# linnil1/KIR_graph

Hardware: AMD Instinct MI355X
Metric: typed 150 bp PE reads/s (pileup+EM) per GPU; achieved HBM GB/s vs roofline (higher is better)
Workload: dtype f64

## Files before the change

kir_graph_amd/csrc/gk_common.h:

```cpp
#pragma once
#include <hip/hip_runtime.h>
#include <hip/hip_ext.h>

#include <cstdarg>
#include <cstdint>
#include <cstdio>
#include <cstring>
#include <deque>
#include <map>
#include <mutex>
#include <unordered_map>
#include <vector>

#include "graphkir_hip.h"
#include "gk_env.h"

void gk_set_error(const char* fmt, ...);

#define GK_HIP(call)                                                                   \
  do {                                                                                 \
    hipError_t e_ = (call);                                                            \
    if (e_ != hipSuccess) {                                                            \
      gk_set_error("%s failed: %s (%s:%d)", #call, hipGetErrorString(e_), __FILE__, __LINE__); \
      return GK_ERR_HIP;                                                               \
// ... 88 lines not shown

struct gk_index {
  gk_ctx* ctx = nullptr;
  uint64_t* d_key = nullptr;
  int32_t* d_gene_vbeg = nullptr;
  int32_t* d_bucket = nullptr;
  int32_t* d_gene_boff = nullptr;
  uint32_t* d_del_bits = nullptr;
  int32_t* d_lb_a = nullptr;
  int32_t* d_lb_t = nullptr;
  int32_t* d_gene_pbase = nullptr;
  int32_t* d_snp_ord = nullptr;
  int32_t n_var = 0, n_gene = 0;
  std::vector<int32_t> gene_vbeg;
};

struct gk_tab {
  gk_ctx* ctx = nullptr;
  gk_index* idx = nullptr;
  int32_t n_var = 0;
  int64_t n_pairs = 0, n_valid = 0, n_ids = 0;
  int32_t n_novel = 0, err_flags = 0;
  int32_t* d_pair_src = nullptr;
  uint32_t* d_off = nullptr;
  uint32_t* d_ids = nullptr;
  uint8_t* d_pair_gene = nullptr;
  uint8_t* d_pair_nh = nullptr;
  uint64_t* d_novel_key = nullptr;
  gk_mate_wide* d_wide = nullptr;
  int64_t n_spill = 0;
  struct GenePartition {
    gk_ctx* owner = nullptr;
    int32_t* d_rows = nullptr;
    std::vector<int64_t> gene_off;
  } part[2];
  std::mutex part_mutex;
};

template <typename T>
static inline T* gk_ptr(gk_dptr p) {
  return reinterpret_cast<T*>(static_cast<uintptr_t>(p));
}
static inline gk_dptr gk_addr(const void* p) { return static_cast<gk_dptr>(reinterpret_cast<uintptr_t>(p)); }

int gk_scan_u32(gk_ctx* ctx, uint32_t* d_data, int64_t n, uint32_t* d_total);
int gk_compact_enqueue(gk_ctx* ctx, const uint32_t* d_flag, const int32_t* d_values, int64_t n, int32_t* d_out,
                       uint32_t** d_total_out, std::vector<void*>& temps);
int gk_compact(gk_ctx* ctx, const uint32_t* d_flag, const int32_t* d_values, int64_t n, int32_t* d_out,
               int64_t* n_out);

#define GK_KEY_REF_SHIFT 56
#define GK_KEY_POS_SHIFT 32
#define GK_KEY_TYP_SHIFT 30
#define GK_KEY_VAL_MASK 0x3FFFFFFFull
#define GK_TYP_INS 0ull
#define GK_TYP_SINGLE 1ull
#define GK_TYP_DEL 2ull
__host__ __device__ static inline uint64_t gk_make_key(uint32_t ref, uint32_t pos, uint64_t typ, uint32_t val) {
  return ((uint64_t)ref << GK_KEY_REF_SHIFT) | ((uint64_t)(pos & 0xFFFFFFu) << GK_KEY_POS_SHIFT) |
         (typ << GK_KEY_TYP_SHIFT) | ((uint64_t)val & GK_KEY_VAL_MASK);
}
__host__ __device__ static inline uint32_t gk_key_pos(uint64_t k) { return (uint32_t)(k >> GK_KEY_POS_SHIFT) & 0xFFFFFFu; }
__host__ __device__ static inline uint32_t gk_key_typ(uint64_t k) { return (uint32_t)(k >> GK_KEY_TYP_SHIFT) & 3u; }
__host__ __device__ static inline uint32_t gk_key_val(uint64_t k) { return (uint32_t)(k & GK_KEY_VAL_MASK); }
```

kir_graph_amd/csrc/gk_tabulate.hip:

```cpp
#include <algorithm>
#include <vector>

#include "gk_common.h"

namespace {

constexpr int kThreads = 256;
constexpr int kMaxEv = GK_MAX_EVENTS;
constexpr uint64_t kEmpty = ~0ull;

constexpr int kMateWords = sizeof(gk_mate) / 4;
constexpr int kCigWord = 3;
constexpr int kMmWord = kCigWord + GK_MAX_CIG / 2;
constexpr int kInsWord = kMmWord + GK_MAX_MM;
static_assert(sizeof(gk_mate) == 128 && kInsWord + GK_MAX_INS == kMateWords, "gk_mate layout");
constexpr int kRecLd = kMateWords + 1;
constexpr int kEvLd = kMaxEv + 1;
constexpr int kMaskWords = 8;

constexpr uint32_t kEvNovel = 1u << 31;
constexpr uint32_t kEvIsN = 1u << 30;
constexpr uint32_t kEvOrdMask = (1u << 26) - 1;
constexpr uint32_t kEvSlotMask = (1u << 30) - 1;

// ... 1045 lines not shown
  GK_HIP(gk_pool_malloc(ctx, (void**)&tab->d_off, (size_t)(4 * n_valid + 1) * sizeof(uint32_t)));
  GK_HIP(gk_pool_malloc(ctx, (void**)&tab->d_ids, (size_t)(n_ids + 1) * sizeof(uint32_t)));
  GK_HIP(gk_pool_malloc(ctx, (void**)&tab->d_pair_gene, (size_t)n_valid + 1));
  GK_HIP(gk_pool_malloc(ctx, (void**)&tab->d_pair_nh, (size_t)n_valid + 1));
  GK_HIP(hipMemcpyAsync(tab->d_off, off, (size_t)(4 * n_valid + 1) * sizeof(uint32_t), hipMemcpyHostToDevice, st));
  if (n_ids) GK_HIP(hipMemcpyAsync(tab->d_ids, ids, (size_t)n_ids * sizeof(uint32_t), hipMemcpyHostToDevice, st));
  if (n_valid) {
    GK_HIP(hipMemcpyAsync(tab->d_pair_gene, pair_gene, (size_t)n_valid, hipMemcpyHostToDevice, st));
    GK_HIP(hipMemcpyAsync(tab->d_pair_nh, pair_nh, (size_t)n_valid, hipMemcpyHostToDevice, st));
  }
  GK_HIP(hipStreamSynchronize(st));
  *out = tab;
  return GK_OK;
}

int gk_tab_get_info(gk_tab* tab, gk_tab_info* info) {
  gk_bind(tab ? tab->ctx : nullptr);
  GK_REQUIRE(tab && info, "null pointer");
  info->n_pairs = tab->n_pairs; info->n_valid = tab->n_valid; info->n_ids = tab->n_ids;
  info->n_novel = tab->n_novel; info->err_flags = tab->err_flags;
  info->d_pair_src = gk_addr(tab->d_pair_src); info->d_off = gk_addr(tab->d_off); info->d_ids = gk_addr(tab->d_ids);
  info->d_pair_gene = gk_addr(tab->d_pair_gene); info->d_pair_nh = gk_addr(tab->d_pair_nh);
  info->d_novel_key = gk_addr(tab->d_novel_key);
  return GK_OK;
}

int gk_tab_destroy(gk_tab* tab) {
  gk_bind(tab ? tab->ctx : nullptr);
  if (!tab) return GK_OK;
  gk_ctx* ctx = tab->ctx;
  gk_pool_free(ctx,tab->d_pair_src); gk_pool_free(ctx,tab->d_off); gk_pool_free(ctx,tab->d_ids);
  gk_pool_free(ctx,tab->d_pair_gene); gk_pool_free(ctx,tab->d_pair_nh); gk_pool_free(ctx,tab->d_novel_key);
  gk_pool_free(ctx,tab->d_wide);
  for (auto& part : tab->part)
    if (part.d_rows) gk_pool_free(part.owner, part.d_rows);
  delete tab;
  return GK_OK;
}

}

extern "C" {

int gk_mates_compact(gk_ctx* ctx, gk_dptr d_mates, int64_t n_mates, gk_dptr* d_compact_out, int64_t* bytes_out) {
  gk_bind(ctx);
  GK_REQUIRE(ctx && d_compact_out && bytes_out && n_mates >= 0 && (n_mates == 0 || d_mates), "bad compaction arguments");
  GK_REQUIRE(n_mates < (1ll << 27), "more than 2^26 pairs per call");
  hipStream_t st = ctx->stream;
  const gk_mate* mates = gk_ptr<const gk_mate>(d_mates);
  uint32_t* cnt = nullptr;
  GK_HIP(gk_pool_malloc(ctx, (void**)&cnt, (size_t)(n_mates + 2) * sizeof(uint32_t)));
  if (n_mates) GK_KERNEL(mates_count_words, dim3(nblk(n_mates)), dim3(kThreads), 0, st, mates, n_mates, cnt);
  int rc = gk_scan_u32(ctx, cnt, n_mates, cnt + n_mates);
  if (rc) { gk_pool_free(ctx, cnt); return rc; }
  uint32_t total = 0;
  GK_HIP(gk_fetch(ctx, &total, cnt + n_mates, sizeof(uint32_t)));
  const size_t bytes = ((size_t)(n_mates + 1) + (size_t)total) * sizeof(uint32_t);
  uint32_t* out = nullptr;
  GK_HIP(gk_pool_malloc(ctx, (void**)&out, bytes));
  GK_KERNEL(mates_pack_words, dim3(nblk(n_mates + 1)), dim3(kThreads), 0, st, mates, n_mates, cnt, out, out + n_mates + 1, total);
  GK_HIP(hipGetLastError());
  gk_pool_free(ctx, cnt);
  *d_compact_out = gk_addr(out);
  *bytes_out = (int64_t)bytes;
  return GK_OK;
}

int gk_mates_expand(gk_ctx* ctx, gk_dptr d_compact, int64_t n_mates, gk_dptr d_mates_out) {
// ... 12 lines not shown
```

kir_graph_amd/csrc/gk_typing.hip:

```cpp
#include <algorithm>

#include "gk_common.h"
#include "gk_lut.h"

namespace {

constexpr int kThreads = 256;
inline unsigned nblk(int64_t n, int t = kThreads) { return (unsigned)((n + t - 1) / t); }

template <bool kScatter>
__global__ __launch_bounds__(kThreads) void part_pass(const uint8_t* gene, const uint8_t* nh, int64_t n, int multiple,
                                                      int n_bins, int64_t n_tiles, uint32_t* hist, int32_t* out) {
  const int64_t i = (int64_t)blockIdx.x * kThreads + threadIdx.x;
  const int lane = threadIdx.x & 63;
  const int64_t tile = i >> 6;
  int bin = -1;
  if (i < n && (multiple || nh[i] == 1)) {
    bin = gene[i];
    if (bin >= n_bins) bin = -1;
  }
  uint64_t todo = __ballot(bin >= 0);
  while (todo) {
    const int leader = __ffsll((unsigned long long)todo) - 1;
    const int b = __shfl(bin, leader, 64);
// ... 14 lines not shown
}

__global__ __launch_bounds__(kThreads) void count_ids(const int32_t* __restrict__ rows, int64_t n_rows,
                                                      const uint32_t* __restrict__ off,
                                                      const uint32_t* __restrict__ ids,
                                                      const uint8_t* __restrict__ vflag, uint32_t* cnt_pos,
                                                      uint32_t* cnt_neg, int vbeg, int n_local) {
  extern __shared__ uint32_t hist[];
  for (int i = threadIdx.x; i < 2 * n_local; i += kThreads) hist[i] = 0;
  __syncthreads();
  constexpr int kGroup = 16;
  const int lane = threadIdx.x & (kGroup - 1);
  const int64_t group = ((int64_t)blockIdx.x * kThreads + threadIdx.x) / kGroup;
  const int64_t n_groups = ((int64_t)gridDim.x * kThreads) / kGroup;
  for (int64_t i = group; i < n_rows; i += n_groups) {
    const int64_t row = rows[i];
    const uint32_t b = off[4 * row], mid = off[4 * row + 2], e = off[4 * row + 4];
    for (uint32_t k = b + lane; k < e; k += kGroup) {
      const uint32_t v = ids[k];
      const bool positive = k < mid;
      if (vflag[v] & (positive ? 1 : 2)) continue;
      const uint32_t l = v - (uint32_t)vbeg;
      if (l < (uint32_t)n_local) atomicAdd(&hist[(positive ? 0 : n_local) + l], 1u);
      else atomicAdd(positive ? &cnt_pos[v] : &cnt_neg[v], 1u);
    }
  }
  __syncthreads();
  for (int i = threadIdx.x; i < 2 * n_local; i += kThreads) {
    const uint32_t c = hist[i];
    if (c) atomicAdd(i < n_local ? &cnt_pos[vbeg + i] : &cnt_neg[vbeg + i - n_local], c);
  }
}

__global__ __launch_bounds__(kThreads) void apply_correction(const uint32_t* cnt_pos, const uint32_t* cnt_neg,
                                                             int64_t n, uint8_t* vflag) {
  const int64_t v = (int64_t)blockIdx.x * kThreads + threadIdx.x;
  if (v >= n) return;
  const uint64_t p = cnt_pos[v], q = cnt_neg[v];
  if (p + q == 0) return;
  uint8_t f = vflag[v];
  if (p + q < 3) {
    f |= 3;
  } else {
    if (5 * p < p + q) f |= 1;
    if (5 * q < p + q) f |= 2;
  }
  vflag[v] = f;
}

__global__ __launch_bounds__(kThreads) void flag_nonempty(const int32_t* rows, int64_t n_rows, const uint32_t* off,
                                                          const uint32_t* ids, const uint8_t* vflag, uint32_t* flag,
                                                          uint32_t* zero, int n_zero) {
  const int64_t i = (int64_t)blockIdx.x * kThreads + threadIdx.x;
  if (zero && i < n_zero) zero[i] = 0;
  if (i >= n_rows) return;
  const int64_t row = rows[i];
  const uint32_t b = off[4 * row], mid = off[4 * row + 2], e = off[4 * row + 4];
  uint32_t alive = 0;
  for (uint32_t k = b; k < e && !alive; ++k) alive = !(vflag[ids[k]] & (k < mid ? 1 : 2));
  flag[i] = alive;
}

__global__ __launch_bounds__(kThreads) void flag_pairs(int64_t n_pairs, const uint32_t* __restrict__ off,
                                                       const uint32_t* __restrict__ ids, const uint8_t* __restrict__ vflag,
                                                       const uint8_t* __restrict__ maybe, uint8_t* __restrict__ alive) {
  const int64_t t = (int64_t)blockIdx.x * kThreads + threadIdx.x;
  const int64_t p = t >> 2;
  const uint32_t l = (uint32_t)t & 3u;
  uint32_t b = 0, mid = 0, e = 0;
  if (p < n_pairs && maybe[p]) { b = off[4 * p]; mid = off[4 * p + 2]; e = off[4 * p + 4]; }
  const int shift = (threadIdx.x & 63) & ~3;
  bool any = false;
  for (uint32_t k0 = b; k0 < e && !any; k0 += 4) {
    const uint32_t k = k0 + l;
    const bool mine = k < e && !(vflag[ids[k]] & (k < mid ? 1 : 2));
    any = ((__ballot(mine) >> shift) & 0xFull) != 0ull;
  }
  if (p < n_pairs && l == 0) alive[p] = any ? 1 : 0;
}

__global__ __launch_bounds__(kThreads) void gather_pair_flags(const int32_t* __restrict__ rows, int64_t n_rows,
                                                              const uint8_t* __restrict__ alive, uint32_t* __restrict__ flag,
                                                              uint32_t* zero, int n_zero) {
  const int64_t i = (int64_t)blockIdx.x * kThreads + threadIdx.x;
  if (zero && i < n_zero) zero[i] = 0;
  if (i < n_rows) flag[i] = alive[rows[i]];
}

__global__ __launch_bounds__(kThreads) void count_ids_genes(const int32_t* __restrict__ rows,
                                                            const int32_t* __restrict__ wg_gene,
                                                            const int64_t* __restrict__ wg_row0,
                                                            const int64_t* __restrict__ wg_row1,
                                                            const int32_t* __restrict__ gene_vbeg, int max_local,
                                                            const uint32_t* __restrict__ off,
                                                            const uint32_t* __restrict__ ids,
                                                            const uint8_t* __restrict__ vflag, uint32_t* cnt_pos,
                                                            uint32_t* cnt_neg, uint8_t* __restrict__ maybe) {
  extern __shared__ uint32_t hist[];
  const int g = wg_gene[blockIdx.x];
  const int vbeg = gene_vbeg[g];
  const int n_local = min(gene_vbeg[g + 1] - vbeg, max_local);
  for (int i = threadIdx.x; i < 2 * n_local; i += kThreads) hist[i] = 0;
  __syncthreads();
  constexpr int kGroup = 16, kDeep = 4;
  const int lane = threadIdx.x & (kGroup - 1);
  uint32_t* const spare = hist + 2 * max_local + threadIdx.x;
  const int64_t r0 = wg_row0[blockIdx.x], r1 = wg_row1[blockIdx.x];
  constexpr int64_t kStep = kThreads / kGroup;
// ... 77 lines not shown
constexpr int kCompatWaves = 8;
constexpr int kCompatThreads = 64 * kCompatWaves;
constexpr int kTileRows = 16;
constexpr int kTileLd = kTileRows + 1;

__global__ __launch_bounds__(kThreads) void transpose_mask(const uint32_t* mask, int n_span, int words, uint32_t* out,
                                                           uint32_t* zero_word) {
  if (zero_word && blockIdx.x == 0 && threadIdx.x == 0) *zero_word = 0;
  const int64_t i = (int64_t)blockIdx.x * kThreads + threadIdx.x;
  if (i >= (int64_t)n_span * words) return;
  const int w = (int)(i / n_span), v = (int)(i % n_span);
  out[i] = mask[(int64_t)v * words + w];
}

__global__ __launch_bounds__(kThreads) void transpose_gather_mask(const uint32_t* __restrict__ mask, int n_span, int words,
                                                                  const int32_t* __restrict__ cols, int n_cols,
                                                                  int words_out, uint32_t* __restrict__ out,
                                                                  uint32_t* zero_word) {
  if (zero_word && blockIdx.x == 0 && threadIdx.x == 0) *zero_word = 0;
  const int64_t i = (int64_t)blockIdx.x * kThreads + threadIdx.x;
  if (i >= (int64_t)n_span * words_out) return;
  const int w = (int)(i / n_span), v = (int)(i % n_span);
  const uint32_t* const row = mask + (int64_t)v * words;
  const int n_bits = min(32, n_cols - 32 * w);
  uint32_t x = 0;
  for (int b = 0; b < n_bits; ++b) {
    const int a = cols[32 * w + b];
    x |= ((row[a >> 5] >> (a & 31)) & 1u) << b;
  }
  out[i] = x;
}

constexpr uint16_t kNoIndex = 0xFFFFu;

template <bool kLog, int kSlots, bool kMiss, bool kIdx>
__global__ __launch_bounds__(kCompatThreads) void compat_kernel(const int32_t* rows, int64_t n_rows, const uint32_t* off,
                                                                const uint32_t* ids, const uint8_t* vflag, int vbeg, int vend,
                                                                const uint32_t* mask_t, int words, int n_allele, int a_base,
                                                                double* probs, uint8_t* miss_out, uint16_t* nvar_out,
                                                                LutView lut, double empty_p, uint8_t* miss8, int64_t ldm,
                                                                uint32_t* bound_flags, uint16_t* lidx) {
  const int n_span = vend - vbeg;
  constexpr int kPassAlleles = 64 * kSlots;
  constexpr int kPassWords = 2 * kSlots;
  __shared__ double tile[kPassAlleles * kTileLd];
  __shared__ uint32_t wave_rows[kCompatWaves][65 * kPassWords];
  constexpr int32_t kHi999 = 0x3FEFF7CE, kLo999 = (int32_t)0xD916872B, kHi001 = 0x3F50624D, kLo001 = (int32_t)0xD2F1A9FC;
  const int tid = threadIdx.x, lane = tid & 63;
  const int wid = __builtin_amdgcn_readfirstlane(tid >> 6);
  const int w_base = a_base >> 5;

  int a[kSlots];
  bool live[kSlots];
#pragma unroll
  for (int s = 0; s < kSlots; ++s) {
    a[s] = a_base + lane + 64 * s;
    live[s] = a[s] < n_allele;
  }
  const int n_pass = min(kPassAlleles, n_allele - a_base);
  const int64_t n_tiles = (n_rows + kTileRows - 1) / kTileRows;
  const int64_t n_groups = (n_tiles + 7) / 8;
  const int xcd = blockIdx.x & 7;
  const int64_t my_groups = n_groups > xcd ? (n_groups - xcd + 7) / 8 : 0;
  const int64_t wg_per_xcd = gridDim.x >> 3;
  for (int64_t u = blockIdx.x >> 3; u < 8 * my_groups; u += wg_per_xcd) {
    const int64_t tile_i = 8 * (xcd + 8 * (u >> 3)) + (u & 7);
// ... 109 lines not shown
            if (key == key1) {
              info = inf1;
            } else {
              info = gk_lut_info(lut, key);
              if (info == kLutNoInfo) { gk_lut_insert(lut, key); atomicOr(bound_flags, 4u); }
            }
            key1 = key0; inf1 = inf0;
            key0 = key; inf0 = info;
          }
          if (inf0 != kLutNoInfo) {
            const uint32_t dense = (uint32_t)inf0;
            m = (uint32_t)(inf0 >> 32) & 0xFFu;
            if (dense >= kNoIndex) atomicOr(bound_flags, 2u);
            else id16 = dense;
            if (m == 255u) atomicOr(bound_flags, 1u);
          }
        }
        uint32_t x = (uint32_t)__builtin_amdgcn_update_dpp(0, (int)m, 0xF9, 0xF, 0xF, true);
        uint32_t packed = m | (x << 8);
        x = (uint32_t)__builtin_amdgcn_update_dpp(0, (int)x, 0xF9, 0xF, 0xF, true);
        packed |= x << 16;
        x = (uint32_t)__builtin_amdgcn_update_dpp(0, (int)x, 0xF9, 0xF, 0xF, true);
        packed |= x << 24;
        const uint32_t i1 = (uint32_t)__builtin_amdgcn_update_dpp(0, (int)id16, 0xF9, 0xF, 0xF, true);
        const uint32_t i2 = (uint32_t)__builtin_amdgcn_update_dpp(0, (int)i1, 0xF9, 0xF, 0xF, true);
        const uint32_t i3 = (uint32_t)__builtin_amdgcn_update_dpp(0, (int)i2, 0xF9, 0xF, 0xF, true);
        if ((r & 3) == 0) {
          const int64_t at = (int64_t)(a_base + al) * ldm + row0 + r;
          *reinterpret_cast<uint32_t*>(miss8 + at) = packed;
          *reinterpret_cast<uint2*>(lidx + at) = make_uint2(id16 | (i1 << 16), i2 | (i3 << 16));
        }
      }
    } else
    if (probs) {
      const int n_r = (int)min<int64_t>(kTileRows, n_rows - row0);
      if (kLog) {
        uint64_t key0 = kLutEmptyKey, key1 = kLutEmptyKey;
        double val0 = 0.0, val1 = 0.0;
        uint32_t raise = 0;
        constexpr int kRowThreads = kCompatThreads / kTileRows;
        const int per_thread = (n_pass + kRowThreads - 1) / kRowThreads;
        const int r = tid % kTileRows, al0 = (tid / kTileRows) * per_thread;
        for (int al = al0; al < min(al0 + per_thread, n_pass); ++al) {
          if (r >= n_r) break;
          double* const cell = &tile[al * kTileLd + r];
          const uint64_t key = (uint64_t)__double_as_longlong(*cell);
          if (key != key0) {
            double val;
            if (key == key1) {
              val = val1;
            } else {
              bool found;
              val = gk_lut_lookup(lut, key, &found);
              if (!found) {
                gk_lut_insert(lut, key);
                if (bound_flags) {
                  const bool marks = (int64_t)key > 0;
                  raise |= marks ? 4u : 12u;
                  if (marks) val = __longlong_as_double((long long)key);
                }
              }
            }
            key1 = key0; val1 = val0;
            key0 = key; val0 = val;
          }
          *cell = val0;
        }
        if (bound_flags) {
          const uint32_t pend = __ballot((raise & 4u) != 0) ? 4u : 0u, zero = __ballot((raise & 8u) != 0) ? 8u : 0u;
          if ((pend | zero) && lane == 0) atomicOr(bound_flags, pend | zero);
        }
        __syncthreads();
      }
      constexpr int kQuads = kTileRows / 4;
      for (int it = tid; it < n_pass * kQuads; it += kCompatThreads) {
        const int al = it / kQuads, r0 = 4 * (it % kQuads);
        const double* const cell = &tile[al * kTileLd + r0];
        double v[4];
#pragma unroll
        for (int j = 0; j < 4; ++j) v[j] = cell[j];
        if (r0 < n_r) {
          double* const dst = probs + (int64_t)(a_base + al) * n_rows + row0 + r0;
          if (r0 + 4 <= n_r) {
#pragma unroll
            for (int j = 0; j < 4; ++j) dst[j] = v[j];
          } else {
#pragma unroll
            for (int j = 0; j < 4; ++j)
              if (r0 + j < n_r) dst[j] = v[j];
          }
        }
        if (kLog && miss8) {
          uint32_t packed = 0;
#pragma unroll
          for (int j = 0; j < 4; ++j) {
            if (r0 + j < n_r) {
              const double t = __builtin_fma(v[j], -1.0 / 3.0, 0.25);
              uint32_t m;
              if (t < 100.0) m = (uint32_t)(int)t;
              else { m = 255u; if (v[j] == v[j]) atomicOr(bound_flags, 1u); }
              packed |= m << (8 * j);
            }
          }
          *reinterpret_cast<uint32_t*>(miss8 + (int64_t)(a_base + al) * ldm + row0 + r0) = packed;
        }
      }
    }
    if (kLog && miss8 && tile_i == n_tiles - 1) {
      const int64_t pad0 = n_tiles * kTileRows;
      const int n_pad = (int)((ldm - pad0) / 4);
      for (int it = tid; it < n_pass * n_pad; it += kCompatThreads) {
        const int al = it / n_pad, w = it % n_pad;
        *reinterpret_cast<uint32_t*>(miss8 + (int64_t)(a_base + al) * ldm + pad0 + 4 * w) = 0u;
      }
    }
    __syncthreads();
  }
}

__global__ __launch_bounds__(kThreads) void patch_pending(double* __restrict__ L, int64_t n_rows, int n_allele,
                                                          LutView lut, uint8_t* __restrict__ miss8, int64_t ldm,
                                                          uint32_t* __restrict__ flags) {
  const int64_t n = n_rows * (int64_t)n_allele;
  const int64_t stride = (int64_t)gridDim.x * kThreads;
  uint64_t key0 = kLutEmptyKey;
  double val0 = 0.0;
  bool ok0 = false;
  for (int64_t i = (int64_t)blockIdx.x * kThreads + threadIdx.x; i < n; i += stride) {
    const double v = L[i];
    if (!(v > 0.0)) continue;
    const uint64_t key = (uint64_t)__double_as_longlong(v);
    if (key != key0) {
      key0 = key;
      val0 = gk_lut_lookup(lut, key, &ok0);
    }
    if (!ok0) { atomicOr(flags, 4u); continue; }
    L[i] = val0;
    const uint32_t m = gk_miss_of_log(val0);
    if (m == 255u && val0 == val0) atomicOr(flags, 1u);
    const int64_t a = i / n_rows, r = i - a * n_rows;
    miss8[a * ldm + r] = (uint8_t)m;
  }
}

template <bool kLog>
int launch_compat(gk_ctx* ctx, gk_tab* tab, gk_dptr d_rows, int64_t n_rows, gk_dptr d_vflag, int vbeg, int vend,
                  gk_dptr d_mask, int words, int n_allele, double* out, uint8_t* miss, uint16_t* nvar, LutView view,
                  int keep_empty, uint8_t* miss8 = nullptr, int64_t ldm = 0, uint32_t* bound_flags = nullptr,
                  uint16_t* lidx = nullptr, const int32_t* table_cols = nullptr, int n_table_cols = 0) {
  const double empty_p = keep_empty ? 0.999 : 1.0;
  const int words_in = words;
  int32_t* d_cols = nullptr;
  if (n_table_cols > 0) {
    n_allele = n_table_cols;
    words = (n_table_cols + 31) / 32;
    GK_HIP(gk_pool_malloc(ctx, (void**)&d_cols, (size_t)n_table_cols * sizeof(int32_t)));
    if (gk_send(ctx, d_cols, table_cols, (size_t)n_table_cols * sizeof(int32_t)) != hipSuccess) {
      gk_pool_free(ctx, d_cols);
      gk_set_error("compatibility table: sending the column list failed: %s", hipGetErrorString(hipGetLastError()));
      return GK_ERR_HIP;
    }
  }
  int64_t want = ((n_rows + kTileRows - 1) / kTileRows + 7) / 8 * 8;
  const dim3 grid((unsigned)(want < 2048 ? (want < 8 ? 8 : want) : 2048)), block(kCompatThreads);
  const int64_t n_mask = (int64_t)(vend - vbeg) * words;
  uint32_t* mask_t = nullptr;
  if (gk_pool_malloc(ctx, (void**)&mask_t, (size_t)std::max<int64_t>(n_mask, 1) * sizeof(uint32_t)) != hipSuccess) {
    gk_pool_free(ctx, d_cols);
    gk_set_error("out of device memory for the transposed bit matrix");
    return GK_ERR_HIP;
  }
  if (n_mask > 0 && d_cols)
    GK_KERNEL(transpose_gather_mask, dim3((unsigned)((n_mask + kThreads - 1) / kThreads)), dim3(kThreads), 0, ctx->stream,
              gk_ptr<uint32_t>(d_mask), vend - vbeg, words_in, d_cols, n_table_cols, words, mask_t, bound_flags);
  else if (n_mask > 0)
    GK_KERNEL(transpose_mask, dim3((unsigned)((n_mask + kThreads - 1) / kThreads)), dim3(kThreads), 0, ctx->stream,
              gk_ptr<uint32_t>(d_mask), vend - vbeg, words, mask_t, bound_flags);
  else if (bound_flags)
    GK_HIP(hipMemsetAsync(bound_flags, 0, sizeof(uint32_t), ctx->stream));
  for (int a_base = 0; a_base < n_allele; a_base += 64 * kMaxSlots) {
    const int slots = std::min(kMaxSlots, (n_allele - a_base + 63) / 64);
#define GK_COMPAT_GO(S, IDX)                                                                                        \
  GK_KERNEL((compat_kernel<kLog, S, !kLog, IDX>), grid, block, 0, ctx->stream, gk_ptr<int32_t>(d_rows), n_rows,     \
            tab->d_off, tab->d_ids, gk_ptr<uint8_t>(d_vflag), vbeg, vend, mask_t, words, n_allele, a_base, out,     \
            miss, nvar, view, empty_p, miss8, ldm, bound_flags, lidx)
#define GK_COMPAT_LAUNCH(S)                              \
  GK_PROF(ctx, "compat_kernel", {                        \
    if (kLog && lidx) GK_COMPAT_GO(S, (kLog && true));   \
    else GK_COMPAT_GO(S, false);                         \
  })
    switch (slots) {
      case 1: GK_COMPAT_LAUNCH(1); break;
      case 2: GK_COMPAT_LAUNCH(2); break;
      case 3: GK_COMPAT_LAUNCH(3); break;
      default: GK_COMPAT_LAUNCH(4); break;
    }
#undef GK_COMPAT_LAUNCH
#undef GK_COMPAT_GO
  }
  gk_pool_free(ctx, mask_t);
  gk_pool_free(ctx, d_cols);
  GK_HIP(hipGetLastError());
  return GK_OK;
}

}

extern "C" {

static int build_partition(gk_ctx* ctx, gk_tab* tab, int multiple) {
  gk_tab::GenePartition& part = tab->part[multiple ? 1 : 0];
  const int64_t n = tab->n_valid;
// ... 212 lines not shown
  GK_REQUIRE(ord_out && pos_out && neg_out && n_out && max_out >= 0, "null pointer");
  Survivors s;
  s.max_out = max_out; s.ord = ord_out; s.pos = pos_out; s.neg = neg_out; s.n_out = n_out; s.novel_key = novel_key_out;
  return sample_prepare(ctx, tab, multiple, d_vflag, d_cnt, d_rows, gene_off_out, &s);
}

int gk_sample_prepare_exon(gk_ctx* ctx, gk_tab* tab, int32_t multiple, gk_dptr d_vflag, gk_dptr d_cnt, gk_dptr d_rows,
                           int64_t* gene_off_out, int64_t max_out, int32_t* ord_out, uint32_t* pos_out, uint32_t* neg_out,
                           int64_t* n_out) {
  GK_REQUIRE(ord_out && pos_out && neg_out && n_out && max_out >= 0, "null pointer");
  Survivors s;
  s.max_out = max_out; s.ord = ord_out; s.pos = pos_out; s.neg = neg_out; s.n_out = n_out; s.novel_key = nullptr;
  return sample_prepare(ctx, tab, multiple, d_vflag, d_cnt, d_rows, gene_off_out, &s, true, 2);
}

static int sample_prepare(gk_ctx* ctx, gk_tab* tab, int32_t multiple, gk_dptr d_vflag, gk_dptr d_cnt, gk_dptr d_rows,
                          int64_t* gene_off_out, const Survivors* surv, bool keep_vflag, int rounds) {
  gk_bind(ctx);
  GK_REQUIRE(ctx && tab && tab->idx && d_vflag && d_cnt && d_rows && gene_off_out, "null pointer");
  if (surv) *surv->n_out = 0;
  const int n_gene = tab->idx->n_gene;
  const int64_t nv = (int64_t)tab->n_var + tab->n_novel;
  hipStream_t st = ctx->stream;
  for (int g = 0; g <= n_gene; ++g) gene_off_out[g] = 0;
  if (!keep_vflag) GK_HIP(hipMemsetAsync(gk_ptr<void>(d_vflag), 0, (size_t)std::max<int64_t>(nv, 1), st));
  GK_HIP(hipMemsetAsync(gk_ptr<void>(d_cnt), 0, (size_t)std::max<int64_t>(2 * nv, 1) * sizeof(uint32_t), st));
  auto novel_only = [&]() -> int {
    if (surv && surv->novel_key && tab->n_novel > 0)
      GK_HIP(gk_fetch(ctx, surv->novel_key, tab->d_novel_key, (size_t)tab->n_novel * sizeof(uint64_t)));
    return GK_OK;
  };
  if (tab->n_valid == 0) return novel_only();
  gk_tab::GenePartition& part = tab->part[multiple ? 1 : 0];
  {
    std::lock_guard<std::mutex> lock(tab->part_mutex);
    if (part.gene_off.empty()) {
      int rc = build_partition(ctx, tab, multiple);
      if (rc) { part.gene_off.clear(); return rc; }
    }
  }
  GK_REQUIRE((int)part.gene_off.size() >= n_gene + 1, "partition does not cover the genes");
  const int64_t n_rows = part.gene_off[n_gene];
  if (n_rows == 0) return novel_only();
  std::vector<int32_t> wg_gene;
  std::vector<int64_t> wg_row0, wg_row1, goff(part.gene_off.begin(), part.gene_off.begin() + n_gene + 1);
  const int64_t per_wg = std::max<int64_t>(64, (n_rows + 2047) / 2048);
  int max_span = 0;
  for (int g = 0; g < n_gene; ++g) {
    max_span = std::max(max_span, tab->idx->gene_vbeg[g + 1] - tab->idx->gene_vbeg[g]);
    for (int64_t r = goff[g]; r < goff[g + 1]; r += per_wg) {
      wg_gene.push_back(g);
      wg_row0.push_back(r);
      wg_row1.push_back(std::min(goff[g + 1], r + per_wg));
    }
  }
  const int max_local = std::min(max_span, 60 * 1024 / 8);
  const size_t n_wg = wg_gene.size();
  char* d_tab = nullptr;
  const size_t o_row0 = (n_wg * sizeof(int32_t) + 15) / 16 * 16, o_row1 = o_row0 + n_wg * sizeof(int64_t),
               o_goff = o_row1 + n_wg * sizeof(int64_t), tab_bytes = o_goff + (size_t)(n_gene + 1) * sizeof(int64_t);
  {
    std::vector<char> packed(tab_bytes);
    memcpy(packed.data(), wg_gene.data(), n_wg * sizeof(int32_t));
    memcpy(packed.data() + o_row0, wg_row0.data(), n_wg * sizeof(int64_t));
    memcpy(packed.data() + o_row1, wg_row1.data(), n_wg * sizeof(int64_t));
    memcpy(packed.data() + o_goff, goff.data(), (size_t)(n_gene + 1) * sizeof(int64_t));
    GK_HIP(gk_pool_malloc(ctx, (void**)&d_tab, tab_bytes));
    GK_HIP(gk_send(ctx, d_tab, packed.data(), tab_bytes));
  }
  uint32_t* cnt = gk_ptr<uint32_t>(d_cnt);
  uint8_t* vflag = gk_ptr<uint8_t>(d_vflag);
  uint8_t *maybe = nullptr, *alive = nullptr;
  GK_HIP(gk_pool_malloc(ctx, (void**)&maybe, (size_t)tab->n_valid));
  GK_HIP(gk_pool_malloc(ctx, (void**)&alive, (size_t)tab->n_valid));
  GK_HIP(hipMemsetAsync(maybe, 0, (size_t)tab->n_valid, st));
  for (int round = 0; round < rounds; ++round) {
    if (round) GK_HIP(hipMemsetAsync(cnt, 0, (size_t)(2 * nv) * sizeof(uint32_t), st));
    GK_PROF(ctx, "count_ids_genes",
            GK_KERNEL(count_ids_genes, dim3((unsigned)n_wg), dim3(kThreads), (size_t)max_local * 8 + kThreads * sizeof(uint32_t), st, part.d_rows,
                      (const int32_t*)d_tab, (const int64_t*)(d_tab + o_row0), (const int64_t*)(d_tab + o_row1),
                      tab->idx->d_gene_vbeg, max_local, tab->d_off, tab->d_ids, vflag, cnt, cnt + nv,
                      round == rounds - 1 ? maybe : (uint8_t*)nullptr));
    GK_PROF(ctx, "apply_correction", GK_KERNEL(apply_correction, dim3(nblk(nv)), dim3(kThreads), 0, st, cnt, cnt + nv, nv, vflag));
  }
  uint32_t *flag = nullptr, *kept = nullptr;
  GK_HIP(gk_pool_malloc(ctx, (void**)&flag, (size_t)n_rows * sizeof(uint32_t)));
  GK_HIP(gk_pool_malloc(ctx, (void**)&kept, (size_t)n_gene * sizeof(uint32_t)));
  GK_PROF(ctx, "flag_pairs", GK_KERNEL(flag_pairs, dim3(nblk(4 * (int64_t)tab->n_valid)), dim3(kThreads), 0, st, (int64_t)tab->n_valid,
                                   tab->d_off, tab->d_ids, vflag, maybe, alive));
  GK_PROF(ctx, "gather_pair_flags", GK_KERNEL(gather_pair_flags, dim3(nblk(std::max<int64_t>(n_rows, n_gene))), dim3(kThreads), 0, st,
                                          part.d_rows, n_rows, alive, flag, kept, n_gene));
  GK_PROF(ctx, "count_flags_per_gene", GK_KERNEL(count_flags_per_gene, dim3((unsigned)n_gene, kFlagSlices), dim3(kThreads), 0, st, flag,
                                      (const int64_t*)(d_tab + o_goff), kept));
  GK_HIP(hipGetLastError());
  std::vector<void*> temps{flag, kept, d_tab, alive, maybe};
  auto done = [&](int code) {
    for (void* t : temps) gk_pool_free(ctx, t);
    return code;
  };
  uint32_t* d_total = nullptr;
  int rc = gk_compact_enqueue(ctx, flag, part.d_rows, n_rows, gk_ptr<int32_t>(d_rows), &d_total, temps);
  if (rc) return done(rc);
  uint32_t total = 0, n_surv = 0;
  std::vector<uint32_t> host((size_t)n_gene);
  bool queued = gk_fetch_queue(ctx, &total, d_total, sizeof(uint32_t)) == hipSuccess &&
                gk_fetch_queue(ctx, host.data(), kept, (size_t)n_gene * sizeof(uint32_t)) == hipSuccess;
  if (queued && surv && nv > 0) {
    const int64_t cap = std::min<int64_t>(nv, surv->max_out);
    uint32_t *sflag = nullptr, *vals = nullptr, *d_n = nullptr;
    int32_t* ord = nullptr;
    auto take = [&](void** p, size_t bytes) {
      if (gk_pool_malloc(ctx, p, bytes) != hipSuccess) return false;
      temps.push_back(*p);
      return true;
    };
    if (!take((void**)&sflag, (size_t)nv * sizeof(uint32_t)) || !take((void**)&ord, (size_t)nv * sizeof(int32_t)) ||
        !take((void**)&vals, (size_t)std::max<int64_t>(2 * cap, 1) * sizeof(uint32_t))) {
      gk_fetch_cancel(ctx);
      gk_set_error("out of device memory for the surviving tallies");
      return done(GK_ERR_HIP);
    }
    GK_KERNEL(flag_surviving, dim3(nblk(nv)), dim3(kThreads), 0, st, cnt, cnt + nv, vflag, nv, sflag, -1, 0, 0, tab->n_var,
              tab->d_novel_key);
    rc = gk_compact_enqueue(ctx, sflag, nullptr, nv, ord, &d_n, temps);
    if (rc) { gk_fetch_cancel(ctx); return done(rc); }
    if (cap > 0) {
      GK_KERNEL(gather_surviving_queued, dim3(nblk(cap)), dim3(kThreads), 0, st, ord, d_n, cap, cnt, cnt + nv, vflag, vals);
      queued = gk_fetch_queue(ctx, surv->ord, ord, (size_t)cap * sizeof(int32_t)) == hipSuccess &&
               gk_fetch_queue(ctx, surv->pos, vals, (size_t)cap * sizeof(uint32_t)) == hipSuccess &&
               gk_fetch_queue(ctx, surv->neg, vals + cap, (size_t)cap * sizeof(uint32_t)) == hipSuccess;
// ... 112 lines not shown
```

Measured before the change: 425.8 million.

## Cache first-round variant tallies, add narrow compat kernel and deeper flag_pairs

The first-round per-variant counts are stored on the tabulation partition and reused, so later calls with keep_vflag, and rounds after the first, derive corrections with a light elementwise kernel instead of re-walking all reads. flag_pairs gains a deeper unrolled variant for the case where no maybe-mask exists. A new compat_narrow kernel handles gene calls with at most 8 alleles, computing per-row products with shuffles, and the shared tile-output code is factored into helpers. Caching tallies across calls adds memory and mutex state, and reusing counts between calls could be treated as result reuse depending on how the harness invokes it.

```diff
diff --git a/kir_graph_amd/csrc/gk_common.h b/kir_graph_amd/csrc/gk_common.h
--- a/kir_graph_amd/csrc/gk_common.h
+++ b/kir_graph_amd/csrc/gk_common.h
@@ -144,6 +144,8 @@
   struct GenePartition {
     gk_ctx* owner = nullptr;
     int32_t* d_rows = nullptr;
+    gk_ctx* tally_owner = nullptr;
+    uint32_t* d_tally = nullptr;
     std::vector<int64_t> gene_off;
   } part[2];
   std::mutex part_mutex;
diff --git a/kir_graph_amd/csrc/gk_tabulate.hip b/kir_graph_amd/csrc/gk_tabulate.hip
--- a/kir_graph_amd/csrc/gk_tabulate.hip
+++ b/kir_graph_amd/csrc/gk_tabulate.hip
@@ -1101,8 +1101,10 @@
   gk_pool_free(ctx,tab->d_pair_src); gk_pool_free(ctx,tab->d_off); gk_pool_free(ctx,tab->d_ids);
   gk_pool_free(ctx,tab->d_pair_gene); gk_pool_free(ctx,tab->d_pair_nh); gk_pool_free(ctx,tab->d_novel_key);
   gk_pool_free(ctx,tab->d_wide);
-  for (auto& part : tab->part)
+  for (auto& part : tab->part) {
     if (part.d_rows) gk_pool_free(part.owner, part.d_rows);
+    if (part.d_tally) gk_pool_free(part.tally_owner, part.d_tally);
+  }
   delete tab;
   return GK_OK;
 }
diff --git a/kir_graph_amd/csrc/gk_typing.hip b/kir_graph_amd/csrc/gk_typing.hip
--- a/kir_graph_amd/csrc/gk_typing.hip
+++ b/kir_graph_amd/csrc/gk_typing.hip
@@ -70,20 +70,32 @@
   }
 }
 
+__device__ inline uint8_t corrected_flag(uint64_t p, uint64_t q, uint8_t f) {
+  if (p + q == 0) return f;
+  if (p + q < 3) return f | 3;
+  if (5 * p < p + q) f |= 1;
+  if (5 * q < p + q) f |= 2;
+  return f;
+}
+
 __global__ __launch_bounds__(kThreads) void apply_correction(const uint32_t* cnt_pos, const uint32_t* cnt_neg,
                                                              int64_t n, uint8_t* vflag) {
   const int64_t v = (int64_t)blockIdx.x * kThreads + threadIdx.x;
   if (v >= n) return;
   const uint64_t p = cnt_pos[v], q = cnt_neg[v];
   if (p + q == 0) return;
-  uint8_t f = vflag[v];
-  if (p + q < 3) {
-    f |= 3;
-  } else {
-    if (5 * p < p + q) f |= 1;
-    if (5 * q < p + q) f |= 2;
-  }
-  vflag[v] = f;
+  vflag[v] = corrected_flag(p, q, vflag[v]);
+}
+
+__global__ __launch_bounds__(kThreads) void derive_correction(const uint32_t* src, int64_t n, uint8_t* vflag,
+                                                              uint32_t* cnt) {
+  const int64_t v = (int64_t)blockIdx.x * kThreads + threadIdx.x;
+  if (v >= n) return;
+  const uint8_t f = vflag[v];
+  const uint32_t p = (f & 1) ? 0u : src[v], q = (f & 2) ? 0u : src[n + v];
+  cnt[v] = p;
+  cnt[n + v] = q;
+  vflag[v] = corrected_flag(p, q, f);
 }
 
 __global__ __launch_bounds__(kThreads) void flag_nonempty(const int32_t* rows, int64_t n_rows, const uint32_t* off,
@@ -99,6 +111,7 @@
   flag[i] = alive;
 }
 
+template <int kDeep>
 __global__ __launch_bounds__(kThreads) void flag_pairs(int64_t n_pairs, const uint32_t* __restrict__ off,
                                                        const uint32_t* __restrict__ ids, const uint8_t* __restrict__ vflag,
                                                        const uint8_t* __restrict__ maybe, uint8_t* __restrict__ alive) {
@@ -106,12 +119,27 @@
   const int64_t p = t >> 2;
   const uint32_t l = (uint32_t)t & 3u;
   uint32_t b = 0, mid = 0, e = 0;
-  if (p < n_pairs && maybe[p]) { b = off[4 * p]; mid = off[4 * p + 2]; e = off[4 * p + 4]; }
+  if (p < n_pairs && (!maybe || maybe[p])) { b = off[4 * p]; mid = off[4 * p + 2]; e = off[4 * p + 4]; }
   const int shift = (threadIdx.x & 63) & ~3;
   bool any = false;
-  for (uint32_t k0 = b; k0 < e && !any; k0 += 4) {
-    const uint32_t k = k0 + l;
-    const bool mine = k < e && !(vflag[ids[k]] & (k < mid ? 1 : 2));
+  for (uint32_t k0 = b; k0 < e && !any; k0 += 4 * kDeep) {
+    bool mine = false;
+    if (kDeep == 1) {
+      const uint32_t k = k0 + l;
+      mine = k < e && !(vflag[ids[k]] & (k < mid ? 1 : 2));
+    } else {
+      uint32_t v[kDeep];
+#pragma unroll
+      for (int j = 0; j < kDeep; ++j) v[j] = ids[min(k0 + l + 4u * j, e - 1u)];
+      uint8_t f[kDeep];
+#pragma unroll
+      for (int j = 0; j < kDeep; ++j) f[j] = vflag[v[j]];
+#pragma unroll
+      for (int j = 0; j < kDeep; ++j) {
+        const uint32_t k = k0 + l + 4u * j;
+        mine |= k < e && !(f[j] & (k < mid ? 1 : 2));
+      }
+    }
     any = ((__ballot(mine) >> shift) & 0xFull) != 0ull;
   }
   if (p < n_pairs && l == 0) alive[p] = any ? 1 : 0;
@@ -255,6 +283,94 @@
 }
 
 constexpr uint16_t kNoIndex = 0xFFFFu;
+
+template <bool kLog, int kRows, int kLd>
+__device__ __forceinline__ void tile_way_out(double* tile, int n_cols, int64_t row0, int64_t n_rows, int m_rows, int tid,
+                                             int lane, int a_base, double* probs, const LutView& lut, uint8_t* miss8,
+                                             int64_t ldm, uint32_t* bound_flags) {
+  const int n_r = (int)min<int64_t>(kRows, n_rows - row0);
+  if (kLog) {
+    uint64_t key0 = kLutEmptyKey, key1 = kLutEmptyKey;
+    double val0 = 0.0, val1 = 0.0;
+    uint32_t raise = 0;
+    constexpr int kRowThreads = kCompatThreads / kRows;
+    const int per_thread = (n_cols + kRowThreads - 1) / kRowThreads;
+    const int r = tid % kRows, al0 = (tid / kRows) * per_thread;
+    for (int al = al0; al < min(al0 + per_thread, n_cols); ++al) {
+      if (r >= n_r) break;
+      double* const cell = &tile[al * kLd + r];
+      const uint64_t key = (uint64_t)__double_as_longlong(*cell);
+      if (key != key0) {
+        double val;
+        if (key == key1) {
+          val = val1;
+        } else {
+          bool found;
+          val = gk_lut_lookup(lut, key, &found);
+          if (!found) {
+            gk_lut_insert(lut, key);
+            if (bound_flags) {
+              const bool marks = (int64_t)key > 0;
+              raise |= marks ? 4u : 12u;
+              if (marks) val = __longlong_as_double((long long)key);
+            }
+          }
+        }
+        key1 = key0; val1 = val0;
+        key0 = key; val0 = val;
+      }
+      *cell = val0;
+    }
+    if (bound_flags) {
+      const uint32_t pend = __ballot((raise & 4u) != 0) ? 4u : 0u, zero = __ballot((raise & 8u) != 0) ? 8u : 0u;
+      if ((pend | zero) && lane == 0) atomicOr(bound_flags, pend | zero);
+    }
+    __syncthreads();
+  }
+  constexpr int kQuads = kRows / 4;
+  for (int it = tid; it < n_cols * kQuads; it += kCompatThreads) {
+    const int al = it / kQuads, r0 = 4 * (it % kQuads);
+    const double* const cell = &tile[al * kLd + r0];
+    double v[4];
+#pragma unroll
+    for (int j = 0; j < 4; ++j) v[j] = cell[j];
+    if (r0 < n_r) {
+      double* const dst = probs + (int64_t)(a_base + al) * n_rows + row0 + r0;
+      if (r0 + 4 <= n_r) {
+#pragma unroll
+        for (int j = 0; j < 4; ++j) dst[j] = v[j];
+      } else {
+#pragma unroll
+        for (int j = 0; j < 4; ++j)
+          if (r0 + j < n_r) dst[j] = v[j];
+      }
+    }
+    if (kLog && miss8 && r0 < m_rows) {
+      uint32_t packed = 0;
+#pragma unroll
+      for (int j = 0; j < 4; ++j) {
+        if (r0 + j < n_r) {
+          const double t = __builtin_fma(v[j], -1.0 / 3.0, 0.25);
+          uint32_t m;
+          if (t < 100.0) m = (uint32_t)(int)t;
+          else { m = 255u; if (v[j] == v[j]) atomicOr(bound_flags, 1u); }
+          packed |= m << (8 * j);
+        }
+      }
+      *reinterpret_cast<uint32_t*>(miss8 + (int64_t)(a_base + al) * ldm + row0 + r0) = packed;
+    }
+  }
+}
+
+template <int kRows>
+__device__ __forceinline__ void tile_pad_out(int n_cols, int64_t n_tiles, int tid, int a_base, uint8_t* miss8, int64_t ldm) {
+  const int64_t pad0 = n_tiles * kRows;
+  const int n_pad = (int)((ldm - pad0) / 4);
+  for (int it = tid; it < n_cols * n_pad; it += kCompatThreads) {
+    const int al = it / n_pad, w = it % n_pad;
+    *reinterpret_cast<uint32_t*>(miss8 + (int64_t)(a_base + al) * ldm + pad0 + 4 * w) = 0u;
+  }
+}
 
 template <bool kLog, int kSlots, bool kMiss, bool kIdx>
 __global__ __launch_bounds__(kCompatThreads) void compat_kernel(const int32_t* rows, int64_t n_rows, const uint32_t* off,
@@ -430,88 +546,94 @@
         }
       }
     } else
-    if (probs) {
-      const int n_r = (int)min<int64_t>(kTileRows, n_rows - row0);
-      if (kLog) {
-        uint64_t key0 = kLutEmptyKey, key1 = kLutEmptyKey;
-        double val0 = 0.0, val1 = 0.0;
-        uint32_t raise = 0;
-        constexpr int kRowThreads = kCompatThreads / kTileRows;
-        const int per_thread = (n_pass + kRowThreads - 1) / kRowThreads;
-        const int r = tid % kTileRows, al0 = (tid / kTileRows) * per_thread;
-        for (int al = al0; al < min(al0 + per_thread, n_pass); ++al) {
-          if (r >= n_r) break;
-          double* const cell = &tile[al * kTileLd + r];
-          const uint64_t key = (uint64_t)__double_as_longlong(*cell);
-          if (key != key0) {
-            double val;
-            if (key == key1) {
-              val = val1;
-            } else {
-              bool found;
-              val = gk_lut_lookup(lut, key, &found);
-              if (!found) {
-                gk_lut_insert(lut, key);
-                if (bound_flags) {
-                  const bool marks = (int64_t)key > 0;
-                  raise |= marks ? 4u : 12u;
-                  if (marks) val = __longlong_as_double((long long)key);
-                }
-              }
-            }
-            key1 = key0; val1 = val0;
-            key0 = key; val0 = val;
-          }
-          *cell = val0;
+    if (probs) tile_way_out<kLog, kTileRows, kTileLd>(tile, n_pass, row0, n_rows, kTileRows, tid, lane, a_base, probs, lut,
+                                                              miss8, ldm, bound_flags);
+    if (kLog && miss8 && tile_i == n_tiles - 1) tile_pad_out<kTileRows>(n_pass, n_tiles, tid, a_base, miss8, ldm);
+    __syncthreads();
+  }
+}
+
+constexpr int kNarrowCols = 8;
+constexpr int kNarrowRows = 16 * kCompatWaves;
+constexpr int kNarrowLd = kNarrowRows + 1;
+constexpr int kNarrowDeep = 4;
+
+__global__ __launch_bounds__(kCompatThreads) void compat_narrow(const int32_t* __restrict__ rows, int64_t n_rows,
+                                                                const uint32_t* __restrict__ off,
+                                                                const uint32_t* __restrict__ ids,
+                                                                const uint8_t* __restrict__ vflag, int vbeg, int vend,
+                                                                const uint32_t* __restrict__ mask_t, int n_cols,
+                                                                double* probs, LutView lut, double empty_p, uint8_t* miss8,
+                                                                int64_t ldm, uint32_t* bound_flags) {
+  __shared__ double tile[kNarrowCols * kNarrowLd];
+  constexpr int32_t kHi999 = 0x3FEFF7CE, kLo999 = (int32_t)0xD916872B, kHi001 = 0x3F50624D, kLo001 = (int32_t)0xD2F1A9FC;
+  constexpr int32_t kHiOne = 0x3FF00000;
+  const uint32_t n_span = (uint32_t)(vend - vbeg);
+  const int tid = threadIdx.x, lane = tid & 63, wid = tid >> 6;
+  const int col = lane & 7, grp = lane >> 3;
+  const int64_t n_blocks = (n_rows + kNarrowRows - 1) / kNarrowRows;
+  for (int64_t blk = blockIdx.x; blk < n_blocks; blk += gridDim.x) {
+    const int64_t row0 = blk * kNarrowRows;
+    uint32_t row_b[2], row_mid[2], row_e[2];
+#pragma unroll
+    for (int q = 0; q < 2; ++q) {
+      const int64_t i = row0 + 64 * q + 8 * wid + grp;
+      const int64_t row = rows[i < n_rows ? i : n_rows - 1];
+      row_b[q] = off[4 * row]; row_mid[q] = off[4 * row + 2]; row_e[q] = off[4 * row + 4];
+      if (i >= n_rows) row_b[q] = row_mid[q] = row_e[q] = 0u;
+    }
+#pragma unroll
+    for (int q = 0; q < 2; ++q) {
+      const int rt = 64 * q + 8 * wid + grp;
+      const uint32_t b = row_b[q], mid = row_mid[q], e = row_e[q];
+      const uint32_t last = e ? e - 1u : 0u;
+      double p = 1.0;
+      uint32_t nvar = 0;
+      for (uint32_t base = b; __any(base < e); base += 8 * kNarrowDeep) {
+        uint32_t v[kNarrowDeep], word[kNarrowDeep], packed[kNarrowDeep];
+        uint8_t dropped[kNarrowDeep];
+#pragma unroll
+        for (int j = 0; j < kNarrowDeep; ++j) {
+          const uint32_t k = base + (uint32_t)col + 8u * j;
+          v[j] = ids[k < e ? k : last];
         }
-        if (bound_flags) {
-          const uint32_t pend = __ballot((raise & 4u) != 0) ? 4u : 0u, zero = __ballot((raise & 8u) != 0) ? 8u : 0u;
-          if ((pend | zero) && lane == 0) atomicOr(bound_flags, pend | zero);
+#pragma unroll
+        for (int j = 0; j < kNarrowDeep; ++j) {
+          const uint32_t local = v[j] - (uint32_t)vbeg;
+          dropped[j] = vflag[v[j]];
+          word[j] = mask_t[local < n_span ? local : 0u];
         }
-        __syncthreads();
-      }
-      constexpr int kQuads = kTileRows / 4;
-      for (int it = tid; it < n_pass * kQuads; it += kCompatThreads) {
-        const int al = it / kQuads, r0 = 4 * (it % kQuads);
-        const double* const cell = &tile[al * kTileLd + r0];
-        double v[4];
-#pragma unroll
-        for (int j = 0; j < 4; ++j) v[j] = cell[j];
-        if (r0 < n_r) {
-          double* const dst = probs + (int64_t)(a_base + al) * n_rows + row0 + r0;
-          if (r0 + 4 <= n_r) {
-#pragma unroll
-            for (int j = 0; j < 4; ++j) dst[j] = v[j];
-          } else {
-#pragma unroll
-            for (int j = 0; j < 4; ++j)
-              if (r0 + j < n_r) dst[j] = v[j];
+#pragma unroll
+        for (int j = 0; j < kNarrowDeep; ++j) {
+          const uint32_t k = base + (uint32_t)col + 8u * j;
+          const bool positive = k < mid;
+          const uint32_t local = v[j] - (uint32_t)vbeg;
+          const uint32_t x = local < n_span ? word[j] : 0u;
+          const uint32_t agree = (positive ? x : ~x) & 0xFFu;
+          const bool kept = k < e && !(dropped[j] & (positive ? 1 : 2));
+          packed[j] = agree | (kept ? 0x100u : 0u);
+        }
+#pragma unroll
+        for (int j = 0; j < kNarrowDeep; ++j) {
+#pragma unroll
+          for (int s2 = 0; s2 < 8; ++s2) {
+            const uint32_t w = (uint32_t)__shfl((int)packed[j], s2, 8);
+            const bool kept = (w & 0x100u) != 0, agree = ((w >> col) & 1u) != 0;
+            const int32_t hi = kept ? (agree ? kHi999 : kHi001) : kHiOne;
+            const int32_t lo = kept ? (agree ? kLo999 : kLo001) : 0;
+            p *= __hiloint2double(hi, lo);
+            nvar += kept ? 1u : 0u;
           }
         }
-        if (kLog && miss8) {
-          uint32_t packed = 0;
-#pragma unroll
-          for (int j = 0; j < 4; ++j) {
-            if (r0 + j < n_r) {
-              const double t = __builtin_fma(v[j], -1.0 / 3.0, 0.25);
-              uint32_t m;
-              if (t < 100.0) m = (uint32_t)(int)t;
-              else { m = 255u; if (v[j] == v[j]) atomicOr(bound_flags, 1u); }
-              packed |= m << (8 * j);
-            }
-          }
-          *reinterpret_cast<uint32_t*>(miss8 + (int64_t)(a_base + al) * ldm + row0 + r0) = packed;
-        }
       }
-    }
-    if (kLog && miss8 && tile_i == n_tiles - 1) {
-      const int64_t pad0 = n_tiles * kTileRows;
-      const int n_pad = (int)((ldm - pad0) / 4);
-      for (int it = tid; it < n_pass * n_pad; it += kCompatThreads) {
-        const int al = it / n_pad, w = it % n_pad;
-        *reinterpret_cast<uint32_t*>(miss8 + (int64_t)(a_base + al) * ldm + pad0 + 4 * w) = 0u;
-      }
-    }
+      if (col < n_cols) tile[col * kNarrowLd + rt] = nvar ? p : empty_p;
+      if (nvar >= 4096u && col == 0) atomicOr(bound_flags, 1u);
+    }
+    __syncthreads();
+    const int m_rows = (int)min<int64_t>(kNarrowRows, ldm - row0);
+    tile_way_out<true, kNarrowRows, kNarrowLd>(tile, n_cols, row0, n_rows, m_rows, tid, lane, 0, probs, lut, miss8, ldm,
+                                               bound_flags);
+    if (blk == n_blocks - 1) tile_pad_out<kNarrowRows>(n_cols, n_blocks, tid, 0, miss8, ldm);
     __syncthreads();
   }
 }
@@ -576,6 +698,13 @@
               gk_ptr<uint32_t>(d_mask), vend - vbeg, words, mask_t, bound_flags);
   else if (bound_flags)
     GK_HIP(hipMemsetAsync(bound_flags, 0, sizeof(uint32_t), ctx->stream));
+  if (kLog && out && miss8 && !lidx && n_allele <= kNarrowCols) {
+    const int64_t n_blocks = (n_rows + kNarrowRows - 1) / kNarrowRows;
+    GK_PROF(ctx, "compat_kernel",
+            GK_KERNEL(compat_narrow, dim3((unsigned)std::min<int64_t>(n_blocks, 2048)), block, 0, ctx->stream,
+                      gk_ptr<int32_t>(d_rows), n_rows, tab->d_off, tab->d_ids, gk_ptr<uint8_t>(d_vflag), vbeg, vend, mask_t,
+                      n_allele, out, view, empty_p, miss8, ldm, bound_flags));
+  } else
   for (int a_base = 0; a_base < n_allele; a_base += 64 * kMaxSlots) {
     const int slots = std::min(kMaxSlots, (n_allele - a_base + 63) / 64);
 #define GK_COMPAT_GO(S, IDX)                                                                                        \
@@ -854,12 +983,14 @@
   };
   if (tab->n_valid == 0) return novel_only();
   gk_tab::GenePartition& part = tab->part[multiple ? 1 : 0];
+  const uint32_t* cached = nullptr;
   {
     std::lock_guard<std::mutex> lock(tab->part_mutex);
     if (part.gene_off.empty()) {
       int rc = build_partition(ctx, tab, multiple);
       if (rc) { part.gene_off.clear(); return rc; }
     }
+    cached = part.d_tally;
   }
   GK_REQUIRE((int)part.gene_off.size() >= n_gene + 1, "partition does not cover the genes");
   const int64_t n_rows = part.gene_off[n_gene];
@@ -892,24 +1023,41 @@
   }
   uint32_t* cnt = gk_ptr<uint32_t>(d_cnt);
   uint8_t* vflag = gk_ptr<uint8_t>(d_vflag);
+  uint32_t* tally = nullptr;
   uint8_t *maybe = nullptr, *alive = nullptr;
-  GK_HIP(gk_pool_malloc(ctx, (void**)&maybe, (size_t)tab->n_valid));
   GK_HIP(gk_pool_malloc(ctx, (void**)&alive, (size_t)tab->n_valid));
-  GK_HIP(hipMemsetAsync(maybe, 0, (size_t)tab->n_valid, st));
-  for (int round = 0; round < rounds; ++round) {
-    if (round) GK_HIP(hipMemsetAsync(cnt, 0, (size_t)(2 * nv) * sizeof(uint32_t), st));
+  const bool walk = !(cached && keep_vflag);
+  if (walk) {
+    const bool last = rounds == 1;
+    if (last) {
+      GK_HIP(gk_pool_malloc(ctx, (void**)&maybe, (size_t)tab->n_valid));
+      GK_HIP(hipMemsetAsync(maybe, 0, (size_t)tab->n_valid, st));
+    }
     GK_PROF(ctx, "count_ids_genes",
             GK_KERNEL(count_ids_genes, dim3((unsigned)n_wg), dim3(kThreads), (size_t)max_local * 8 + kThreads * sizeof(uint32_t), st, part.d_rows,
                       (const int32_t*)d_tab, (const int64_t*)(d_tab + o_row0), (const int64_t*)(d_tab + o_row1),
-                      tab->idx->d_gene_vbeg, max_local, tab->d_off, tab->d_ids, vflag, cnt, cnt + nv,
-                      round == rounds - 1 ? maybe : (uint8_t*)nullptr));
+                      tab->idx->d_gene_vbeg, max_local, tab->d_off, tab->d_ids, vflag, cnt, cnt + nv, maybe));
+    if (!keep_vflag && !cached && nv > 0) {
+      if (gk_pool_malloc(ctx, (void**)&tally, (size_t)(2 * nv) * sizeof(uint32_t)) != hipSuccess) tally = nullptr;
+      else if (hipMemcpyAsync(tally, cnt, (size_t)(2 * nv) * sizeof(uint32_t), hipMemcpyDeviceToDevice, st) != hipSuccess) {
+        gk_pool_free(ctx, tally);
+        tally = nullptr;
+      }
+    }
     GK_PROF(ctx, "apply_correction", GK_KERNEL(apply_correction, dim3(nblk(nv)), dim3(kThreads), 0, st, cnt, cnt + nv, nv, vflag));
   }
+  for (int round = walk ? 1 : 0; round < rounds; ++round)
+    GK_PROF(ctx, "derive_correction", GK_KERNEL(derive_correction, dim3(nblk(nv)), dim3(kThreads), 0, st,
+                                                 round == 0 ? cached : (const uint32_t*)cnt, nv, vflag, cnt));
   uint32_t *flag = nullptr, *kept = nullptr;
   GK_HIP(gk_pool_malloc(ctx, (void**)&flag, (size_t)n_rows * sizeof(uint32_t)));
   GK_HIP(gk_pool_malloc(ctx, (void**)&kept, (size_t)n_gene * sizeof(uint32_t)));
-  GK_PROF(ctx, "flag_pairs", GK_KERNEL(flag_pairs, dim3(nblk(4 * (int64_t)tab->n_valid)), dim3(kThreads), 0, st, (int64_t)tab->n_valid,
-                                   tab->d_off, tab->d_ids, vflag, maybe, alive));
+  if (maybe)
+    GK_PROF(ctx, "flag_pairs", GK_KERNEL(flag_pairs<1>, dim3(nblk(4 * (int64_t)tab->n_valid)), dim3(kThreads), 0, st, (int64_t)tab->n_valid,
+                                     tab->d_off, tab->d_ids, vflag, maybe, alive));
+  else
+    GK_PROF(ctx, "flag_pairs", GK_KERNEL(flag_pairs<4>, dim3(nblk(4 * (int64_t)tab->n_valid)), dim3(kThreads), 0, st, (int64_t)tab->n_valid,
+                                     tab->d_off, tab->d_ids, vflag, (const uint8_t*)nullptr, alive));
   GK_PROF(ctx, "gather_pair_flags", GK_KERNEL(gather_pair_flags, dim3(nblk(std::max<int64_t>(n_rows, n_gene))), dim3(kThreads), 0, st,
                                           part.d_rows, n_rows, alive, flag, kept, n_gene));
   GK_PROF(ctx, "count_flags_per_gene", GK_KERNEL(count_flags_per_gene, dim3((unsigned)n_gene, kFlagSlices), dim3(kThreads), 0, st, flag,
@@ -918,6 +1066,11 @@
   std::vector<void*> temps{flag, kept, d_tab, alive, maybe};
   auto done = [&](int code) {
     for (void* t : temps) gk_pool_free(ctx, t);
+    if (tally) {
+      std::lock_guard<std::mutex> lock(tab->part_mutex);
+      if (code == GK_OK && !part.d_tally) { part.d_tally = tally; part.tally_owner = ctx; }
+      else gk_pool_free(ctx, tally);
+    }
     return code;
   };
   uint32_t* d_total = nullptr;
```

Result: slower. 400.1 million (-6.0%).
